# alazarteka/Self-Forcing

Measured on AMD Instinct MI355X. Metric: decoded frames/sec/node, Wan-1.3B 832x480 4-step AR rollout, higher is better.
Workload: dtype bf16

## Files before the change

### self-forcing_amd/csrc/gemm_bf16.hip

```cpp
#include <type_traits>
#include "sf_common.h"
#include "lds_dma.h"
#include "../../include/sf_hip.h"

namespace {

constexpr int BM = 128, BN = 128, BK = 64;
constexpr int GEMM_THREADS = 256;
constexpr int TILE_BYTES = BM * BK * 2;
constexpr int STAGE_BYTES = 2 * TILE_BYTES;
constexpr int GEMM_LDS = 2 * STAGE_BYTES;

struct GemmP {
  const bf16_t* a;
  const bf16_t* w;
  const bf16_t* bias;
  bf16_t* out;
  const bf16_t* resid;
  const bf16_t* gate_mod;
  const bf16_t* gate_e0;
  long gate_group_stride;
  int rows_per_group;
  int M, N, K, lda, ldw, ldo, ldr;
  int tiles_m, tiles_n;
  long a_bs, w_bs, o_bs, r_bs;
  const float* a_scale;
  const float* w_scale;
  int rows_per_seg;
};

typedef int i32x4 __attribute__((ext_vector_type(4)));
typedef int i32x8 __attribute__((ext_vector_type(8)));

__device__ __forceinline__ f32x4 mfma_f8(const bf16x8& w0, const bf16x8& w1, const bf16x8& x0, const bf16x8& x1, const f32x4& acc) {
  const i32x8 wv = __builtin_shufflevector(__builtin_bit_cast(i32x4, w0), __builtin_bit_cast(i32x4, w1), 0, 1, 2, 3, 4, 5, 6, 7);
  const i32x8 xv = __builtin_shufflevector(__builtin_bit_cast(i32x4, x0), __builtin_bit_cast(i32x4, x1), 0, 1, 2, 3, 4, 5, 6, 7);
  return __builtin_amdgcn_mfma_scale_f32_16x16x128_f8f6f4(wv, xv, acc, 0, 0, 0, 127, 0, 127);
}

template <int MT>
__device__ __forceinline__ void fp8_scale_acc(const GemmP& p, f32x4 (&acc)[MT][4], int m_base, int n_base, int lane) {
  f32x4 ws[4];
#pragma unroll
  for (int nt = 0; nt < 4; ++nt) ws[nt] = *reinterpret_cast<const f32x4*>(p.w_scale + min(n_base + nt * 16 + (lane >> 4) * 4, p.N - 4));
#pragma unroll
  for (int mt = 0; mt < MT; ++mt) {
    const float sa = p.a_scale[min(m_base + mt * 16 + (lane & 15), p.M - 1) / p.rows_per_seg];
#pragma unroll
    for (int nt = 0; nt < 4; ++nt)
#pragma unroll
      for (int j = 0; j < 4; ++j) acc[mt][nt][j] = acc[mt][nt][j] * (sa * ws[nt][j]);
  }
}

template <int EPI>
__device__ __forceinline__ bf16x4 epi_apply(const GemmP& p, const f32x4& a4, int m, int n, const bf16_t* e0row) {
  float y[4];
#pragma unroll
  for (int j = 0; j < 4; ++j) y[j] = a4[j];
  if (p.bias) {
    const bf16x4 b = *reinterpret_cast<const bf16x4*>(p.bias + n);
#pragma unroll
    for (int j = 0; j < 4; ++j) y[j] += (float)b[j];
  }
  if (EPI == SF_EPI_BIAS_GELU) {
#pragma unroll
    for (int j = 0; j < 4; ++j) y[j] = gelu_tanh_f(y[j]);
  }
  if (EPI == SF_EPI_BIAS_GATE_RESID) {
    const bf16x4 gm = *reinterpret_cast<const bf16x4*>(p.gate_mod + n);
    const bf16x4 ge = *reinterpret_cast<const bf16x4*>(e0row + n);
#pragma unroll
    for (int j = 0; j < 4; ++j) y[j] *= (float)(bf16_t)((float)gm[j] + (float)ge[j]);
  }
  if (EPI == SF_EPI_BIAS_RESID || EPI == SF_EPI_BIAS_GATE_RESID) {
    const bf16x4 rv = *reinterpret_cast<const bf16x4*>(p.resid + (long)m * p.ldr + n);
#pragma unroll
    for (int j = 0; j < 4; ++j) y[j] += (float)rv[j];
  }
  bf16x4 o;
#pragma unroll
  for (int j = 0; j < 4; ++j) o[j] = (bf16_t)y[j];
  return o;
}

template <int EPI, int MT>
__device__ __forceinline__ void gemm_epilogue(const GemmP& p, f32x4 (&acc)[MT][4], int mrow, int ncol) {
#pragma unroll
  for (int mt = 0; mt < MT; ++mt) {
    const int m = mrow + mt * 16;
    if (m >= p.M) continue;
    const bf16_t* e0row = nullptr;
    if (EPI == SF_EPI_BIAS_GATE_RESID) e0row = p.gate_e0 + (long)(m / p.rows_per_group) * p.gate_group_stride;
#pragma unroll
    for (int nt = 0; nt < 4; ++nt) {
      const int n = ncol + nt * 16;
      if (n >= p.N) continue;
      if (EPI == SF_EPI_F32) {
        *reinterpret_cast<f32x4*>(reinterpret_cast<float*>(p.out) + (long)m * p.ldo + n) = acc[mt][nt];
        continue;
      }
      *reinterpret_cast<bf16x4*>(p.out + (long)m * p.ldo + n) = epi_apply<EPI>(p, acc[mt][nt], m, n, e0row);
    }
  }
}

template <int EPI>
__device__ __forceinline__ bf16x4 epi_math(const f32x4& a4, const bf16x4& b, const bf16x4& gm, const bf16x4& ge, const bf16x4& rv) {
  float y[4];
#pragma unroll
  for (int j = 0; j < 4; ++j) y[j] = a4[j] + (float)b[j];
  if (EPI == SF_EPI_BIAS_GELU) {
#pragma unroll
    for (int j = 0; j < 4; ++j) y[j] = gelu_tanh_f(y[j]);
  }
  if (EPI == SF_EPI_BIAS_GATE_RESID) {
#pragma unroll
    for (int j = 0; j < 4; ++j) y[j] *= (float)(bf16_t)((float)gm[j] + (float)ge[j]);
  }
  if (EPI == SF_EPI_BIAS_RESID || EPI == SF_EPI_BIAS_GATE_RESID) {
#pragma unroll
    for (int j = 0; j < 4; ++j) y[j] += (float)rv[j];
  }
  bf16x4 o;
#pragma unroll
  for (int j = 0; j < 4; ++j) o[j] = (bf16_t)y[j];
  return o;
}

template <int EPI, int MT>
__device__ __forceinline__ void gemm_epilogue_lds(const GemmP& p, f32x4 (&acc)[MT][4], int m_base, int n_base, char* wbuf, int lane) {
  const int r16 = lane & 15, cg = lane >> 4;
  constexpr bool GATE = EPI == SF_EPI_BIAS_GATE_RESID;
  constexpr bool RESID = EPI == SF_EPI_BIAS_RESID || EPI == SF_EPI_BIAS_GATE_RESID;
  const bf16x4 zero4 = {(bf16_t)0.f, (bf16_t)0.f, (bf16_t)0.f, (bf16_t)0.f};
  int ncol[4];
  bf16x4 bias_v[4], gm_v[4];
#pragma unroll
  for (int nt = 0; nt < 4; ++nt) {
    ncol[nt] = min(n_base + nt * 16 + cg * 4, p.N - 4);
    bias_v[nt] = zero4;
    gm_v[nt] = zero4;
  }
  if (p.bias) {
#pragma unroll
    for (int nt = 0; nt < 4; ++nt) bias_v[nt] = *reinterpret_cast<const bf16x4*>(p.bias + ncol[nt]);
  }
  if (GATE) {
#pragma unroll
    for (int nt = 0; nt < 4; ++nt) gm_v[nt] = *reinterpret_cast<const bf16x4*>(p.gate_mod + ncol[nt]);
  }
  constexpr int MB = 4;
#pragma unroll
  for (int m0 = 0; m0 < MT; m0 += MB) {
    bf16x4 rv[MB][4], ge[MB][4];
#pragma unroll
    for (int i = 0; i < MB; ++i) {
      if (m0 + i >= MT) break;
      const int m = min(m_base + (m0 + i) * 16 + r16, p.M - 1);
      const bf16_t* e0row = GATE ? p.gate_e0 + (long)(m / p.rows_per_group) * p.gate_group_stride : nullptr;
#pragma unroll
      for (int nt = 0; nt < 4; ++nt) {
        rv[i][nt] = RESID ? *reinterpret_cast<const bf16x4*>(p.resid + (long)m * p.ldr + ncol[nt]) : zero4;
        ge[i][nt] = GATE ? *reinterpret_cast<const bf16x4*>(e0row + ncol[nt]) : zero4;
      }
    }
#pragma unroll
    for (int i = 0; i < MB; ++i) {
      if (m0 + i >= MT) break;
      const int row = (m0 + i) * 16 + r16;
#pragma unroll
      for (int nt = 0; nt < 4; ++nt) {
        const int col = nt * 16 + cg * 4;
        const bf16x4 o = epi_math<EPI>(acc[m0 + i][nt], bias_v[nt], gm_v[nt], ge[i][nt], rv[i][nt]);
        const int chunk = (col >> 3) ^ (row & 7);
        *reinterpret_cast<bf16x4*>(wbuf + row * 128 + (chunk << 4) + (col & 4) * 2) = o;
      }
    }
  }
  __builtin_amdgcn_s_waitcnt(0xc07f);
  const int rr = lane >> 3, ch = lane & 7;
#pragma unroll
  for (int i = 0; i < 2 * MT; ++i) {
    const int row = i * 8 + rr;
    const int m = m_base + row, n = n_base + ch * 8;
    const bf16x8 v = *reinterpret_cast<const bf16x8*>(wbuf + row * 128 + ((ch ^ (row & 7)) << 4));
    if (m < p.M && n < p.N) *reinterpret_cast<bf16x8*>(p.out + (long)m * p.ldo + n) = v;
  }
}

template <int EPI, bool F8>
__global__ __launch_bounds__(GEMM_THREADS, 2) void gemm_bf16_kernel(GemmP p) {
  extern __shared__ __attribute__((aligned(16))) char smem[];
  const int tid = threadIdx.x;
  const int lane = tid & 63;
  const int wave = __builtin_amdgcn_readfirstlane(tid >> 6);

  if (blockIdx.y) {
    const long bz = blockIdx.y;
    p.a += bz * p.a_bs; p.w += bz * p.w_bs;
    if (EPI == SF_EPI_F32) p.out = reinterpret_cast<bf16_t*>(reinterpret_cast<float*>(p.out) + bz * p.o_bs); else p.out += bz * p.o_bs;
    if (p.resid) p.resid += bz * p.r_bs;
  }
  const int nwg = gridDim.x, bid = blockIdx.x;
  const int wg = sf_xcd_remap(bid, nwg);
  constexpr int GROUP_M = 8;
  const int width = GROUP_M * p.tiles_n;
  const int group = wg / width, first_m = group * GROUP_M;
  const int gsz = min(p.tiles_m - first_m, GROUP_M);
  const int in_group = wg - group * width;
  const int tm = first_m + in_group % gsz, tn = in_group / gsz;
  const int m0 = tm * BM, n0 = tn * BN;

  const bf16_t* a_src[4];
  const bf16_t* w_src[4];
#pragma unroll
  for (int i = 0; i < 4; ++i) {
    const int r = (wave * 4 + i) * 8 + (lane >> 3);
    const int c = (lane & 7) ^ ((r >> 1) & 7);
    const int am = min(m0 + r, p.M - 1);
    const int wn = min(n0 + r, p.N - 1);
    a_src[i] = p.a + (long)am * p.lda + c * 8;
    w_src[i] = p.w + (long)wn * p.ldw + c * 8;
  }
  auto stage = [&](int buf, int kt) {
    char* base = smem + buf * STAGE_BYTES + wave * 4096;
    const int k0 = kt * BK;
#pragma unroll
    for (int i = 0; i < 4; ++i) glds16(a_src[i] + k0, base + i * 1024);
#pragma unroll
    for (int i = 0; i < 4; ++i) glds16(w_src[i] + k0, base + TILE_BYTES + i * 1024);
  };

  const int wr = wave >> 1, wc = wave & 1;
  const int i16 = lane & 15, kq = lane >> 4;
  const int swz = (i16 >> 1) & 7;
  const int x_row_off = (wr * 64 + i16) * 128;
  const int w_row_off = TILE_BYTES + (wc * 64 + i16) * 128;
  const int coff0 = ((0 + kq) ^ swz) << 4;
  const int coff1 = ((4 + kq) ^ swz) << 4;

  f32x4 acc[4][4];
#pragma unroll
  for (int i = 0; i < 4; ++i)
#pragma unroll
    for (int j = 0; j < 4; ++j) acc[i][j] = f32x4{0.f, 0.f, 0.f, 0.f};

  const int nk = p.K / BK;
  stage(0, 0);
  __builtin_amdgcn_s_waitcnt(0);
  __syncthreads();

  for (int kt = 0; kt < nk; ++kt) {
    const int cur = kt & 1;
    const char* buf = smem + cur * STAGE_BYTES;
    const int kn = min(kt + 1, nk - 1) * BK;
    char* sbase = smem + (cur ^ 1) * STAGE_BYTES + wave * 4096;
    bf16x8 xf0[4], wf0[4], xf1[4], wf1[4];
    if constexpr (F8) {
#pragma unroll
      for (int t = 0; t < 4; ++t) {
        xf0[t] = *reinterpret_cast<const bf16x8*>(buf + x_row_off + t * 2048 + coff0);
        wf0[t] = *reinterpret_cast<const bf16x8*>(buf + w_row_off + t * 2048 + coff0);
        xf1[t] = *reinterpret_cast<const bf16x8*>(buf + x_row_off + t * 2048 + coff1);
        wf1[t] = *reinterpret_cast<const bf16x8*>(buf + w_row_off + t * 2048 + coff1);
      }
      __builtin_amdgcn_sched_barrier(0);
#pragma unroll
      for (int i = 0; i < 8; ++i) {
        const int mt = i >> 1, nt0 = (i & 1) * 2;
        acc[mt][nt0] = mfma_f8(wf0[nt0], wf1[nt0], xf0[mt], xf1[mt], acc[mt][nt0]);
        acc[mt][nt0 + 1] = mfma_f8(wf0[nt0 + 1], wf1[nt0 + 1], xf0[mt], xf1[mt], acc[mt][nt0 + 1]);
        if (i < 4) glds16(a_src[i] + kn, sbase + i * 1024);
        else glds16(w_src[i - 4] + kn, sbase + TILE_BYTES + (i - 4) * 1024);
        __builtin_amdgcn_sched_barrier(0);
      }
      __syncthreads();
      continue;
    }
#pragma unroll
    for (int t = 0; t < 4; ++t) {
      xf0[t] = *reinterpret_cast<const bf16x8*>(buf + x_row_off + t * 2048 + coff0);
      wf0[t] = *reinterpret_cast<const bf16x8*>(buf + w_row_off + t * 2048 + coff0);
    }
    __builtin_amdgcn_sched_barrier(0);
#pragma unroll
    for (int i = 0; i < 8; ++i) {
      const int mt = i >> 1, nt0 = (i & 1) * 2;
      acc[mt][nt0] = __builtin_amdgcn_mfma_f32_16x16x32_bf16(wf0[nt0], xf0[mt], acc[mt][nt0], 0, 0, 0);
      acc[mt][nt0 + 1] = __builtin_amdgcn_mfma_f32_16x16x32_bf16(wf0[nt0 + 1], xf0[mt], acc[mt][nt0 + 1], 0, 0, 0);
      if (i < 4) {
        xf1[i] = *reinterpret_cast<const bf16x8*>(buf + x_row_off + i * 2048 + coff1);
        glds16(a_src[i] + kn, sbase + i * 1024);
      } else {
        wf1[i - 4] = *reinterpret_cast<const bf16x8*>(buf + w_row_off + (i - 4) * 2048 + coff1);
        glds16(w_src[i - 4] + kn, sbase + TILE_BYTES + (i - 4) * 1024);
      }
      __builtin_amdgcn_sched_barrier(0);
    }
#pragma unroll
    for (int mt = 0; mt < 4; ++mt)
#pragma unroll
      for (int nt = 0; nt < 4; ++nt)
        acc[mt][nt] = __builtin_amdgcn_mfma_f32_16x16x32_bf16(wf1[nt], xf1[mt], acc[mt][nt], 0, 0, 0);
    __builtin_amdgcn_sched_barrier(0);
    __syncthreads();
  }

  if constexpr (F8) fp8_scale_acc<4>(p, acc, m0 + wr * 64, n0 + wc * 64, lane);
  const int mrow = m0 + wr * 64 + (lane & 15);
  const int ncol = n0 + wc * 64 + (lane >> 4) * 4;
  if (EPI != SF_EPI_F32 && (p.N & 7) == 0 && (p.ldo & 7) == 0)
    gemm_epilogue_lds<EPI, 4>(p, acc, m0 + wr * 64, n0 + wc * 64, smem + wave * 8192, lane);
  else
    gemm_epilogue<EPI, 4>(p, acc, mrow, ncol);
}


constexpr int PP_THREADS = 512;

template <int MT>
struct PPCfg {
  static constexpr int BM = 32 * MT;
  static constexpr int A_BYTES = BM * 128;
  static constexpr int B_BYTES = 256 * 128;
  static constexpr int STAGE = A_BYTES + B_BYTES;
  static constexpr int LDS = 2 * STAGE;
  static constexpr int PA = (2 * MT + 7) / 8;
};

template <int EPI, int MT, bool F8>
__global__ __launch_bounds__(PP_THREADS) void gemm_pp_kernel(GemmP p) {
  using Cfg = PPCfg<MT>;
  constexpr int BMp = Cfg::BM, PA = Cfg::PA;
  constexpr int HQA = (MT + 1) / 2, HQB = MT / 2;
  extern __shared__ __attribute__((aligned(16))) char smem[];
  const int tid = threadIdx.x;
  const int lane = tid & 63;
  const int wave = __builtin_amdgcn_readfirstlane(tid >> 6);
  const int grp = wave >> 2, wc = wave & 3;

  const int nwg = gridDim.x, bid = blockIdx.x;
  const int wg = sf_xcd_remap(bid, nwg);
  constexpr int GROUP_M = MT >= 6 ? 4 : 8;
  const int width = GROUP_M * p.tiles_n;
  const int group = wg / width, first_m = group * GROUP_M;
  const int gsz = min(p.tiles_m - first_m, GROUP_M);
  const int in_group = wg - group * width;
  const int tm = first_m + in_group % gsz, tn = in_group / gsz;
  const int m0 = tm * BMp, n0 = tn * 256;

  const bf16_t* a_src[2][PA];
  const bf16_t* w_src[2][2];
#pragma unroll
  for (int h = 0; h < 2; ++h) {
#pragma unroll
    for (int i = 0; i < PA; ++i) {
      const int r = h * (BMp / 2) + (wave + 8 * i) * 8 + (lane >> 3);
      const int c = (lane & 7) ^ ((r >> 1) & 7);
      a_src[h][i] = p.a + (long)min(m0 + r, p.M - 1) * p.lda + c * 8;
    }
#pragma unroll
    for (int i = 0; i < 2; ++i) {
      const int r = h * 128 + (wave + 8 * i) * 8 + (lane >> 3);
      const int c = (lane & 7) ^ ((r >> 1) & 7);
      w_src[h][i] = p.w + (long)min(n0 + r, p.N - 1) * p.ldw + c * 8;
    }
  }
  auto dma_a = [&](int h, int kt) {
    char* base = smem + (kt & 1) * Cfg::STAGE + h * (Cfg::A_BYTES / 2) + wave * 1024;
#pragma unroll
    for (int i = 0; i < PA; ++i)
      if (wave + 8 * i < 2 * MT) glds16(a_src[h][i] + kt * BK, base + i * 8192);
  };
  auto dma_b = [&](int h, int kt) {
    char* base = smem + (kt & 1) * Cfg::STAGE + Cfg::A_BYTES + h * (Cfg::B_BYTES / 2) + wave * 1024;
#pragma unroll
    for (int i = 0; i < 2; ++i) glds16(w_src[h][i] + kt * BK, base + i * 8192);
  };

  const int i16 = lane & 15, kq = lane >> 4;
  const int swz = (i16 >> 1) & 7;
  const int x_row_off = (grp * (BMp / 2) + i16) * 128;
  const int w_row_off = Cfg::A_BYTES + (wc * 64 + i16) * 128;
  const int coff[2] = {((0 + kq) ^ swz) << 4, ((4 + kq) ^ swz) << 4};

  f32x4 acc[MT][4];
#pragma unroll
  for (int i = 0; i < MT; ++i)
#pragma unroll
    for (int j = 0; j < 4; ++j) acc[i][j] = f32x4{0.f, 0.f, 0.f, 0.f};
  bf16x8 af[HQA][2], bfr[4][2];

#ifdef SF_STAMP
  unsigned long long* stamp = (EPI == SF_EPI_BIAS && p.gate_e0) ? reinterpret_cast<unsigned long long*>(const_cast<bf16_t*>(p.gate_e0)) + ((long)bid * 2 + grp) * 8 : nullptr;
  if (stamp && (tid & 255) == 0) { stamp[0] = __builtin_amdgcn_s_memtime(); stamp[4] = __builtin_amdgcn_s_memrealtime(); }
#endif
  const int nk = p.K / BK;
  dma_a(0, 0); dma_a(1, 0); dma_b(0, 0); dma_b(1, 0);
  if (nk > 1) { dma_b(0, 1); dma_b(1, 1); asm volatile("s_waitcnt vmcnt(4)" ::: "memory"); }
  else asm volatile("s_waitcnt vmcnt(0)" ::: "memory");
  __builtin_amdgcn_s_barrier();
#ifdef SF_STAMP
  if (stamp && (tid & 255) == 0) stamp[1] = __builtin_amdgcn_s_memtime();
#endif
  if (grp == 1) __builtin_amdgcn_s_barrier();

  auto end_load_segment = [&]() {
    __builtin_amdgcn_s_waitcnt(0xc07f);
    __builtin_amdgcn_sched_barrier(0);
    __builtin_amdgcn_s_barrier();
    __builtin_amdgcn_sched_barrier(0);
  };
  auto cluster = [&](auto qc, int c0) {
    constexpr int q = decltype(qc)::value, NQ = q == 0 ? HQA : HQB;
    __builtin_amdgcn_s_setprio(1);
    if constexpr (F8) {
#pragma unroll
      for (int mt = 0; mt < NQ; ++mt)
#pragma unroll
        for (int nt = 0; nt < 2; ++nt)
          acc[q * HQA + mt][c0 + nt] = mfma_f8(bfr[c0 + nt][0], bfr[c0 + nt][1], af[mt][0], af[mt][1], acc[q * HQA + mt][c0 + nt]);
    } else {
#pragma unroll
      for (int ks = 0; ks < 2; ++ks)
#pragma unroll
        for (int mt = 0; mt < NQ; ++mt)
#pragma unroll
          for (int nt = 0; nt < 2; ++nt)
            acc[q * HQA + mt][c0 + nt] = __builtin_amdgcn_mfma_f32_16x16x32_bf16(bfr[c0 + nt][ks], af[mt][ks], acc[q * HQA + mt][c0 + nt], 0, 0, 0);
    }
    __builtin_amdgcn_s_setprio(0);
    __builtin_amdgcn_sched_barrier(0);
    __builtin_amdgcn_s_barrier();
    __builtin_amdgcn_sched_barrier(0);
  };
  auto read_a = [&](const char* buf, auto qc) {
    constexpr int q = decltype(qc)::value, NQ = q == 0 ? HQA : HQB;
#pragma unroll
    for (int mt = 0; mt < NQ; ++mt)
#pragma unroll
      for (int ks = 0; ks < 2; ++ks)
        af[mt][ks] = *reinterpret_cast<const bf16x8*>(buf + x_row_off + (q * HQA + mt) * 2048 + coff[ks]);
  };
  auto read_b = [&](const char* buf, int c0) {
#pragma unroll
    for (int nt = 0; nt < 2; ++nt)
#pragma unroll
      for (int ks = 0; ks < 2; ++ks)
        bfr[c0 + nt][ks] = *reinterpret_cast<const bf16x8*>(buf + w_row_off + (c0 + nt) * 2048 + coff[ks]);
  };

  constexpr std::integral_constant<int, 0> Q0{};
  constexpr std::integral_constant<int, 1> Q1{};
  for (int kt = 0; kt < nk; ++kt) {
    const char* buf = smem + (kt & 1) * Cfg::STAGE;
    const bool more1 = kt + 1 < nk, more2 = kt + 2 < nk;
    read_a(buf, Q0);
    read_b(buf, 0);
    if (more1) dma_a(0, kt + 1);
    end_load_segment();
    cluster(Q0, 0);
    read_b(buf, 2);
    if (more1) dma_a(1, kt + 1);
    end_load_segment();
    cluster(Q0, 2);
    read_a(buf, Q1);
    if (more2) dma_b(0, kt + 2);
    end_load_segment();
    cluster(Q1, 2);
    if (more2) {
      dma_b(1, kt + 2);
      asm volatile("s_waitcnt vmcnt(4)" ::: "memory");
    } else {
      asm volatile("s_waitcnt vmcnt(0)" ::: "memory");
    }
    end_load_segment();
    cluster(Q1, 0);
  }
  if (grp == 0) __builtin_amdgcn_s_barrier();
#ifdef SF_STAMP
  if (stamp && (tid & 255) == 0) stamp[2] = __builtin_amdgcn_s_memtime();
#endif

  const int m_base = m0 + grp * (BMp / 2), n_base = n0 + wc * 64;
  if constexpr (F8) fp8_scale_acc<MT>(p, acc, m_base, n_base, lane);
  if ((p.N & 7) == 0 && (p.ldo & 7) == 0)
    gemm_epilogue_lds<EPI, MT>(p, acc, m_base, n_base, smem + wave * (MT * 2048), lane);
  else
    gemm_epilogue<EPI, MT>(p, acc, m_base + (lane & 15), n_base + (lane >> 4) * 4);
#ifdef SF_STAMP
  asm volatile("s_waitcnt vmcnt(0)" ::: "memory");
  if (stamp && (tid & 255) == 0) { stamp[3] = __builtin_amdgcn_s_memtime(); stamp[5] = __builtin_amdgcn_s_memrealtime(); }
#endif
}

constexpr int PP2_A = 128 * 128, PP2_B = 256 * 128;
constexpr int PP2_LDS = 3 * (PP2_A + PP2_B);

template <int EPI, bool F8>
__global__ __launch_bounds__(PP_THREADS) void gemm_pp2_kernel(GemmP p) {
  extern __shared__ __attribute__((aligned(16))) char smem[];
  const int tid = threadIdx.x;
  const int lane = tid & 63;
  const int wave = __builtin_amdgcn_readfirstlane(tid >> 6);
  const int grp = wave >> 2, wc = wave & 3;

  const int nwg = gridDim.x, bid = blockIdx.x;
  const int wg = sf_xcd_remap(bid, nwg);
  constexpr int GROUP_M = 8;
  const int width = GROUP_M * p.tiles_n;
  const int group = wg / width, first_m = group * GROUP_M;
  const int gsz = min(p.tiles_m - first_m, GROUP_M);
  const int in_group = wg - group * width;
  const int tm = first_m + in_group % gsz, tn = in_group / gsz;
  const int m0 = tm * 128, n0 = tn * 256;

  const bf16_t* a_src[2];
  const bf16_t* w_src[4];
#pragma unroll
  for (int i = 0; i < 2; ++i) {
    const int r = (wave + 8 * i) * 8 + (lane >> 3);
    a_src[i] = p.a + (long)min(m0 + r, p.M - 1) * p.lda + ((lane & 7) ^ ((r >> 1) & 7)) * 8;
  }
#pragma unroll
  for (int i = 0; i < 4; ++i) {
    const int r = (wave + 8 * i) * 8 + (lane >> 3);
    w_src[i] = p.w + (long)min(n0 + r, p.N - 1) * p.ldw + ((lane & 7) ^ ((r >> 1) & 7)) * 8;
  }
  auto dma_a = [&](int slot, int kt) {
    char* base = smem + slot * PP2_A + wave * 1024;
#pragma unroll
    for (int i = 0; i < 2; ++i) glds16(a_src[i] + kt * BK, base + i * 8192);
  };
  auto dma_b = [&](int slot, int kt) {
    char* base = smem + 3 * PP2_A + slot * PP2_B + wave * 1024;
#pragma unroll
    for (int i = 0; i < 4; ++i) glds16(w_src[i] + kt * BK, base + i * 8192);
  };

  const int i16 = lane & 15, kq = lane >> 4;
  const int swz = (i16 >> 1) & 7;
  const int x_row_off = (grp * 64 + i16) * 128;
  const int w_row_off = 3 * PP2_A + (wc * 64 + i16) * 128;
  const int coff[2] = {((0 + kq) ^ swz) << 4, ((4 + kq) ^ swz) << 4};

  f32x4 acc[4][4];
#pragma unroll
  for (int i = 0; i < 4; ++i)
#pragma unroll
    for (int j = 0; j < 4; ++j) acc[i][j] = f32x4{0.f, 0.f, 0.f, 0.f};
  bf16x8 af[4][2], bfr[4][2];

  const int nk = p.K / BK;
  dma_a(0, 0); dma_b(0, 0);
  if (nk > 1) { dma_a(1, 1); dma_b(1, 1); asm volatile("s_waitcnt vmcnt(6)" ::: "memory"); }
  else asm volatile("s_waitcnt vmcnt(0)" ::: "memory");
  __builtin_amdgcn_s_barrier();
  if (grp == 1) __builtin_amdgcn_s_barrier();

  auto end_load_segment = [&]() {
    __builtin_amdgcn_s_waitcnt(0xc07f);
    __builtin_amdgcn_sched_barrier(0);
    __builtin_amdgcn_s_barrier();
    __builtin_amdgcn_sched_barrier(0);
  };
  auto cluster = [&](int c0) {
    __builtin_amdgcn_s_setprio(1);
    if constexpr (F8) {
#pragma unroll
      for (int mt = 0; mt < 4; ++mt)
#pragma unroll
        for (int nt = 0; nt < 2; ++nt)
          acc[mt][c0 + nt] = mfma_f8(bfr[c0 + nt][0], bfr[c0 + nt][1], af[mt][0], af[mt][1], acc[mt][c0 + nt]);
    } else {
#pragma unroll
      for (int ks = 0; ks < 2; ++ks)
#pragma unroll
        for (int mt = 0; mt < 4; ++mt)
#pragma unroll
          for (int nt = 0; nt < 2; ++nt)
            acc[mt][c0 + nt] = __builtin_amdgcn_mfma_f32_16x16x32_bf16(bfr[c0 + nt][ks], af[mt][ks], acc[mt][c0 + nt], 0, 0, 0);
    }
    __builtin_amdgcn_s_setprio(0);
    __builtin_amdgcn_sched_barrier(0);
    __builtin_amdgcn_s_barrier();
    __builtin_amdgcn_sched_barrier(0);
  };

  int slot = 0;
  for (int kt = 0; kt < nk; ++kt) {
    const char* abuf = smem + slot * PP2_A;
    const char* bbuf = smem + slot * PP2_B;
    const int nslot = slot == 0 ? 2 : slot - 1;
    const bool more2 = kt + 2 < nk;
#pragma unroll
    for (int mt = 0; mt < 4; ++mt)
#pragma unroll
      for (int ks = 0; ks < 2; ++ks) af[mt][ks] = *reinterpret_cast<const bf16x8*>(abuf + x_row_off + mt * 2048 + coff[ks]);
#pragma unroll
    for (int nt = 0; nt < 2; ++nt)
#pragma unroll
      for (int ks = 0; ks < 2; ++ks) bfr[nt][ks] = *reinterpret_cast<const bf16x8*>(bbuf + w_row_off + nt * 2048 + coff[ks]);
    if (more2) dma_a(nslot, kt + 2);
    end_load_segment();
    cluster(0);
#pragma unroll
    for (int nt = 2; nt < 4; ++nt)
#pragma unroll
      for (int ks = 0; ks < 2; ++ks) bfr[nt][ks] = *reinterpret_cast<const bf16x8*>(bbuf + w_row_off + nt * 2048 + coff[ks]);
    if (more2) {
      dma_b(nslot, kt + 2);
      asm volatile("s_waitcnt vmcnt(6)" ::: "memory");
    } else {
      asm volatile("s_waitcnt vmcnt(0)" ::: "memory");
    }
    end_load_segment();
    cluster(2);
    slot = slot == 2 ? 0 : slot + 1;
  }
  if (grp == 0) __builtin_amdgcn_s_barrier();

  const int m_base = m0 + grp * 64, n_base = n0 + wc * 64;
  if constexpr (F8) fp8_scale_acc<4>(p, acc, m_base, n_base, lane);
  if ((p.N & 7) == 0 && (p.ldo & 7) == 0)
    gemm_epilogue_lds<EPI, 4>(p, acc, m_base, n_base, smem + wave * 8192, lane);
  else
    gemm_epilogue<EPI, 4>(p, acc, m_base + (lane & 15), n_base + (lane >> 4) * 4);
}

template <int EPI, bool F8>
int launch_pp2(GemmP& p, hipStream_t s) {
  static bool attr = false;
  if (!attr) {
    (void)hipFuncSetAttribute(reinterpret_cast<const void*>(&gemm_pp2_kernel<EPI, F8>), hipFuncAttributeMaxDynamicSharedMemorySize, PP2_LDS);
    attr = true;
  }
  p.tiles_m = (p.M + 127) / 128;
  p.tiles_n = (p.N + 255) / 256;
  hipLaunchKernelGGL((gemm_pp2_kernel<EPI, F8>), dim3(p.tiles_m * p.tiles_n), dim3(PP_THREADS), PP2_LDS, s, p);
  return 0;
}

template <bool F8>
int launch_pp2_epi(GemmP& p, int epilogue, hipStream_t s) {
  switch (epilogue) {
    case SF_EPI_BIAS: return launch_pp2<SF_EPI_BIAS, F8>(p, s);
    case SF_EPI_BIAS_GELU: return launch_pp2<SF_EPI_BIAS_GELU, F8>(p, s);
    case SF_EPI_BIAS_RESID: return launch_pp2<SF_EPI_BIAS_RESID, F8>(p, s);
    case SF_EPI_BIAS_GATE_RESID: return launch_pp2<SF_EPI_BIAS_GATE_RESID, F8>(p, s);
    default: return -1;
  }
}

template <int EPI, int MT, bool F8>
int launch_pp(GemmP& p, hipStream_t s) {
  using Cfg = PPCfg<MT>;
  static bool attr = false;
  if (!attr) {
    (void)hipFuncSetAttribute(reinterpret_cast<const void*>(&gemm_pp_kernel<EPI, MT, F8>), hipFuncAttributeMaxDynamicSharedMemorySize, Cfg::LDS);
    attr = true;
  }
  p.tiles_m = (p.M + Cfg::BM - 1) / Cfg::BM;
  p.tiles_n = (p.N + 255) / 256;
  hipLaunchKernelGGL((gemm_pp_kernel<EPI, MT, F8>), dim3(p.tiles_m * p.tiles_n), dim3(PP_THREADS), Cfg::LDS, s, p);
  return 0;
}

template <int MT, bool F8>
int launch_pp_epi(GemmP& p, int epilogue, hipStream_t s) {
  switch (epilogue) {
    case SF_EPI_BIAS: return launch_pp<SF_EPI_BIAS, MT, F8>(p, s);
    case SF_EPI_BIAS_GELU: return launch_pp<SF_EPI_BIAS_GELU, MT, F8>(p, s);
    case SF_EPI_BIAS_RESID: return launch_pp<SF_EPI_BIAS_RESID, MT, F8>(p, s);
    case SF_EPI_BIAS_GATE_RESID: return launch_pp<SF_EPI_BIAS_GATE_RESID, MT, F8>(p, s);
    default: return -1;
  }
}

int check_args(const sf_gemm_args* a, const char* name, int bk) {
  SF_CHECK(a != nullptr, "%s: null args", name);
  SF_CHECK(a->M > 0 && a->N > 0 && a->K > 0, "%s: empty problem M=%d N=%d K=%d", name, a->M, a->N, a->K);
  SF_CHECK(a->K % bk == 0, "%s: K=%d must be a multiple of %d", name, a->K, bk);
  SF_CHECK(a->N % 4 == 0, "%s: N=%d must be a multiple of 4", name, a->N);
  SF_CHECK(a->lda % (bk / 8) == 0 && a->ldw % (bk / 8) == 0 && a->ldo % 4 == 0, "%s: lda/ldw must be multiples of %d, ldo of 4", name, bk / 8);
  SF_CHECK(a->lda >= a->K && a->ldw >= a->K && a->ldo >= a->N, "%s: leading dimension too small", name);
  SF_CHECK(a->a && a->w && a->out, "%s: null tensor", name);
  SF_CHECK(((uintptr_t)a->a % 16 == 0) && ((uintptr_t)a->w % 16 == 0) && ((uintptr_t)a->out % 8 == 0), "%s: misaligned tensor", name);
  if (a->epilogue == SF_EPI_BIAS_RESID || a->epilogue == SF_EPI_BIAS_GATE_RESID) {
    SF_CHECK(a->resid != nullptr && a->ldr >= a->N && a->ldr % 4 == 0, "%s: residual epilogue needs resid/ldr", name);
  }
  if (a->epilogue == SF_EPI_BIAS_GATE_RESID) {
    SF_CHECK(a->gate_mod && a->gate_e0 && a->rows_per_group > 0, "%s: gate epilogue needs gate_mod/gate_e0/rows_per_group", name);
  }
  SF_CHECK(a->structure >= SF_GEMM_AUTO && a->structure <= SF_GEMM_PP192, "%s: unknown structure %d", name, a->structure);
  return 0;
}

template <bool F8>
int run_gemm(const sf_gemm_args* a, GemmP& p, const char* name, hipStream_t s) {
  int st = a->structure;
  const int nk = p.K / BK;
  const bool pp_ok = a->batch <= 1 && a->epilogue != SF_EPI_F32 && nk >= 2;
  if (st == SF_GEMM_AUTO) {
    st = SF_GEMM_T128;
    if (pp_ok && a->M >= 1024 && a->N >= 1024 && a->K >= 512) {
      static const struct { int st, rows; double rel; } cand[] = {
          {SF_GEMM_PP256, 256, 1.00}, {SF_GEMM_PP224, 224, 1.02}, {SF_GEMM_PP192, 192, 1.05}, {SF_GEMM_PP128, 128, 1.14}};
      const long tn = (a->N + 255) / 256;
      double best = 1e30;
      for (const auto& c : cand) {
        const long tiles = (long)((a->M + c.rows - 1) / c.rows) * tn;
        const double cost = (double)((tiles + 255) / 256) * (c.rows / 256.0 * c.rel + 0.04);
        if (cost < best - 1e-9) { best = cost; st = c.st; }
      }
    }
  }
  const bool is_pp = st == SF_GEMM_PP256 || st == SF_GEMM_PP224 || st == SF_GEMM_PP192 || st == SF_GEMM_PP128;
  if (is_pp && !pp_ok) st = SF_GEMM_T128;
  else if (is_pp) {
    const int rc = st == SF_GEMM_PP256 ? launch_pp_epi<8, F8>(p, a->epilogue, s)
                 : st == SF_GEMM_PP224 ? launch_pp_epi<7, F8>(p, a->epilogue, s)
                 : st == SF_GEMM_PP192 ? launch_pp_epi<6, F8>(p, a->epilogue, s) : launch_pp2_epi<F8>(p, a->epilogue, s);
    SF_CHECK(rc == 0, "%s: unknown epilogue %d", name, a->epilogue);
    SF_HIP_LAUNCH_CHECK(name);
    return 0;
  }
  const int batch = a->batch > 1 ? a->batch : 1;
  p.a_bs = a->a_bstride; p.w_bs = a->w_bstride; p.o_bs = a->o_bstride; p.r_bs = a->r_bstride;
  SF_CHECK(batch == 1 || (a->a_bstride % 8 == 0 && a->w_bstride % 8 == 0 && a->o_bstride % 4 == 0 && a->r_bstride % 4 == 0),
           "%s: batch strides must keep 16-byte (operands) / 8-byte (output) alignment", name);
  const dim3 grid(p.tiles_m * p.tiles_n, batch), block(GEMM_THREADS);
  switch (a->epilogue) {
    case SF_EPI_BIAS: hipLaunchKernelGGL((gemm_bf16_kernel<SF_EPI_BIAS, F8>), grid, block, GEMM_LDS, s, p); break;
    case SF_EPI_BIAS_GELU: hipLaunchKernelGGL((gemm_bf16_kernel<SF_EPI_BIAS_GELU, F8>), grid, block, GEMM_LDS, s, p); break;
    case SF_EPI_BIAS_RESID: hipLaunchKernelGGL((gemm_bf16_kernel<SF_EPI_BIAS_RESID, F8>), grid, block, GEMM_LDS, s, p); break;
    case SF_EPI_BIAS_GATE_RESID: hipLaunchKernelGGL((gemm_bf16_kernel<SF_EPI_BIAS_GATE_RESID, F8>), grid, block, GEMM_LDS, s, p); break;
    case SF_EPI_F32:
      if constexpr (F8) {
        SF_CHECK(false, "%s: the raw fp32 epilogue is bf16-only", name);
      } else {
        SF_CHECK((uintptr_t)a->out % 16 == 0, "%s: fp32 output must be 16-byte aligned", name);
        hipLaunchKernelGGL((gemm_bf16_kernel<SF_EPI_F32, false>), grid, block, GEMM_LDS, s, p);
      }
      break;
    default: SF_CHECK(false, "%s: unknown epilogue %d", name, a->epilogue);
  }
  SF_HIP_LAUNCH_CHECK(name);
  return 0;
}

void fill_params(const sf_gemm_args* a, GemmP& p, int unit) {
  p.a = (const bf16_t*)a->a; p.w = (const bf16_t*)a->w; p.bias = (const bf16_t*)a->bias;
  p.out = (bf16_t*)a->out; p.resid = (const bf16_t*)a->resid;
  p.gate_mod = (const bf16_t*)a->gate_mod; p.gate_e0 = (const bf16_t*)a->gate_e0;
  p.gate_group_stride = a->gate_group_stride; p.rows_per_group = a->rows_per_group;
  p.M = a->M; p.N = a->N; p.K = a->K / unit; p.lda = a->lda / unit; p.ldw = a->ldw / unit; p.ldo = a->ldo; p.ldr = a->ldr;
  p.tiles_n = (a->N + BN - 1) / BN;
  p.tiles_m = (a->M + BM - 1) / BM;
  p.a_scale = nullptr; p.w_scale = nullptr; p.rows_per_seg = 1;
}

}

extern "C" int sf_gemm_bf16(const sf_gemm_args* a, void* stream) {
  if (const int rc = check_args(a, "sf_gemm_bf16", BK)) return rc;
  GemmP p;
  fill_params(a, p, 1);
  return run_gemm<false>(a, p, "sf_gemm_bf16", (hipStream_t)stream);
}

extern "C" int sf_gemm_fp8(const sf_gemm_args* a, const float* a_scale, int rows_per_segment, const float* w_scale, void* stream) {
  if (const int rc = check_args(a, "sf_gemm_fp8", 2 * BK)) return rc;
  SF_CHECK(a->batch <= 1, "sf_gemm_fp8: batched products are bf16-only");
  SF_CHECK(a_scale && w_scale && rows_per_segment > 0, "sf_gemm_fp8: needs a_scale, w_scale and rows_per_segment > 0");
  SF_CHECK((uintptr_t)w_scale % 16 == 0, "sf_gemm_fp8: w_scale must be 16-byte aligned");
  GemmP p;
  fill_params(a, p, 2);
  p.a_scale = a_scale; p.w_scale = w_scale; p.rows_per_seg = rows_per_segment;
  return run_gemm<true>(a, p, "sf_gemm_fp8", (hipStream_t)stream);
}
```

Before: 93.76.

## Prefetch GEMM epilogue operands during final K-tile and hoist gate computation

Bias, gate and residual loads for the LDS epilogue are now issued early: column operands before the K loop, and residual rows in place of DMA slots during the peeled last K iteration. This hides epilogue global-load latency behind the final MFMAs. The gate (mod + e0) is formed once per row group instead of once per row, with a loop over groups when a tile spans several. The cost is higher register pressure and more template and scheduling complexity (opaque asm, sched barriers).

```diff
diff --git a/self-forcing_amd/csrc/gemm_bf16.hip b/self-forcing_amd/csrc/gemm_bf16.hip
--- a/self-forcing_amd/csrc/gemm_bf16.hip
+++ b/self-forcing_amd/csrc/gemm_bf16.hip
@@ -32,6 +32,14 @@
 typedef int i32x4 __attribute__((ext_vector_type(4)));
 typedef int i32x8 __attribute__((ext_vector_type(8)));
 
+template <int N, int I = 0, class F>
+__device__ __forceinline__ void static_for(F&& f) {
+  if constexpr (I < N) {
+    f(std::integral_constant<int, I>{});
+    static_for<N, I + 1>(f);
+  }
+}
+
 __device__ __forceinline__ f32x4 mfma_f8(const bf16x8& w0, const bf16x8& w1, const bf16x8& x0, const bf16x8& x1, const f32x4& acc) {
   const i32x8 wv = __builtin_shufflevector(__builtin_bit_cast(i32x4, w0), __builtin_bit_cast(i32x4, w1), 0, 1, 2, 3, 4, 5, 6, 7);
   const i32x8 xv = __builtin_shufflevector(__builtin_bit_cast(i32x4, x0), __builtin_bit_cast(i32x4, x1), 0, 1, 2, 3, 4, 5, 6, 7);
@@ -106,7 +114,7 @@
 }
 
 template <int EPI>
-__device__ __forceinline__ bf16x4 epi_math(const f32x4& a4, const bf16x4& b, const bf16x4& gm, const bf16x4& ge, const bf16x4& rv) {
+__device__ __forceinline__ bf16x4 epi_math(const f32x4& a4, const bf16x4& b, const bf16x4& g, const bf16x4& rv) {
   float y[4];
 #pragma unroll
   for (int j = 0; j < 4; ++j) y[j] = a4[j] + (float)b[j];
@@ -116,7 +124,7 @@
   }
   if (EPI == SF_EPI_BIAS_GATE_RESID) {
 #pragma unroll
-    for (int j = 0; j < 4; ++j) y[j] *= (float)(bf16_t)((float)gm[j] + (float)ge[j]);
+    for (int j = 0; j < 4; ++j) y[j] *= (float)g[j];
   }
   if (EPI == SF_EPI_BIAS_RESID || EPI == SF_EPI_BIAS_GATE_RESID) {
 #pragma unroll
@@ -128,55 +136,139 @@
   return o;
 }
 
+__device__ __forceinline__ void opaque(f32x4& v) { asm volatile("" : "+v"(v)); }
+__device__ __forceinline__ void opaque(bf16x4& v) {
+  unsigned long long t = __builtin_bit_cast(unsigned long long, v);
+  asm volatile("" : "+v"(t));
+  v = __builtin_bit_cast(bf16x4, t);
+}
+
+__device__ __forceinline__ bf16x4 epi_gate(const bf16x4& gm, const bf16x4& ge) {
+  bf16x4 g;
+#pragma unroll
+  for (int j = 0; j < 4; ++j) g[j] = (bf16_t)((float)gm[j] + (float)ge[j]);
+  return g;
+}
+
 template <int EPI, int MT>
-__device__ __forceinline__ void gemm_epilogue_lds(const GemmP& p, f32x4 (&acc)[MT][4], int m_base, int n_base, char* wbuf, int lane) {
+struct EpiOps {
+  static constexpr bool GATE = EPI == SF_EPI_BIAS_GATE_RESID;
+  static constexpr bool RESID = EPI == SF_EPI_BIAS_RESID || EPI == SF_EPI_BIAS_GATE_RESID;
+  int ncol[4];
+  bf16x4 bias[4];
+  bf16x4 gate[4];
+  bf16x4 ge[4];
+  bf16x4 rv[MT][4];
+  int g_first, g_last;
+};
+
+template <int EPI, int MT>
+__device__ __forceinline__ void epi_request_cols(const GemmP& p, EpiOps<EPI, MT>& e, int m_base, int n_base, int lane) {
+  const bf16x4 zero4 = {(bf16_t)0.f, (bf16_t)0.f, (bf16_t)0.f, (bf16_t)0.f};
+  const int cg = lane >> 4;
+#pragma unroll
+  for (int nt = 0; nt < 4; ++nt) {
+    e.ncol[nt] = min(n_base + nt * 16 + cg * 4, p.N - 4);
+    e.bias[nt] = zero4;
+    e.gate[nt] = zero4;
+  }
+  e.g_first = e.g_last = 0;
+  if constexpr (!EpiOps<EPI, MT>::RESID) {
+#pragma unroll
+    for (int b = 0; b < MT; ++b)
+#pragma unroll
+      for (int nt = 0; nt < 4; ++nt) e.rv[b][nt] = zero4;
+  }
+  if (p.bias) {
+#pragma unroll
+    for (int nt = 0; nt < 4; ++nt) e.bias[nt] = *reinterpret_cast<const bf16x4*>(p.bias + e.ncol[nt]);
+  }
+  if constexpr (EpiOps<EPI, MT>::GATE) {
+#pragma unroll
+    for (int nt = 0; nt < 4; ++nt) e.gate[nt] = *reinterpret_cast<const bf16x4*>(p.gate_mod + e.ncol[nt]);
+    e.g_first = min(m_base, p.M - 1) / p.rows_per_group;
+    e.g_last = min(m_base + 16 * MT - 1, p.M - 1) / p.rows_per_group;
+    const bf16_t* e0row = p.gate_e0 + (long)e.g_first * p.gate_group_stride;
+#pragma unroll
+    for (int nt = 0; nt < 4; ++nt) e.ge[nt] = *reinterpret_cast<const bf16x4*>(e0row + e.ncol[nt]);
+  }
+}
+
+template <int EPI, int MT>
+__device__ __forceinline__ void epi_form_gate(EpiOps<EPI, MT>& e) {
+  if constexpr (EpiOps<EPI, MT>::GATE) {
+#pragma unroll
+    for (int nt = 0; nt < 4; ++nt) e.gate[nt] = epi_gate(e.gate[nt], e.ge[nt]);
+  }
+#pragma unroll
+  for (int nt = 0; nt < 4; ++nt) opaque(e.bias[nt]);
+}
+
+template <int B0, int B1, int EPI, int MT>
+__device__ __forceinline__ void epi_request_rows(const GemmP& p, EpiOps<EPI, MT>& e, int m_base, int lane) {
+  if constexpr (EpiOps<EPI, MT>::RESID) {
+#pragma unroll
+    for (int b = B0; b < (B1 < MT ? B1 : MT); ++b) {
+      const bf16_t* rrow = p.resid + (long)min(m_base + b * 16 + (lane & 15), p.M - 1) * p.ldr;
+#pragma unroll
+      for (int nt = 0; nt < 4; ++nt) e.rv[b][nt] = *reinterpret_cast<const bf16x4*>(rrow + e.ncol[nt]);
+    }
+  }
+}
+
+template <int MT, bool F8> struct EpiPlan {
+  static constexpr bool EARLY = !(F8 && MT == 8);
+  static constexpr int PRE = !EARLY ? 4 : (MT == 8 || (F8 && MT == 7)) ? 2 : MT < 4 ? MT : 4, HALF = (PRE + 1) / 2;
+  static constexpr int WIN = EARLY ? MT : 4;
+};
+
+template <int EPI, int MT, int PRE, int WIN = MT>
+__device__ __forceinline__ void gemm_epilogue_lds(const GemmP& p, f32x4 (&acc)[MT][4], EpiOps<EPI, MT>& e, int m_base, int n_base, char* wbuf, int lane) {
   const int r16 = lane & 15, cg = lane >> 4;
-  constexpr bool GATE = EPI == SF_EPI_BIAS_GATE_RESID;
-  constexpr bool RESID = EPI == SF_EPI_BIAS_RESID || EPI == SF_EPI_BIAS_GATE_RESID;
-  const bf16x4 zero4 = {(bf16_t)0.f, (bf16_t)0.f, (bf16_t)0.f, (bf16_t)0.f};
-  int ncol[4];
-  bf16x4 bias_v[4], gm_v[4];
-#pragma unroll
-  for (int nt = 0; nt < 4; ++nt) {
-    ncol[nt] = min(n_base + nt * 16 + cg * 4, p.N - 4);
-    bias_v[nt] = zero4;
-    gm_v[nt] = zero4;
-  }
-  if (p.bias) {
-#pragma unroll
-    for (int nt = 0; nt < 4; ++nt) bias_v[nt] = *reinterpret_cast<const bf16x4*>(p.bias + ncol[nt]);
-  }
-  if (GATE) {
-#pragma unroll
-    for (int nt = 0; nt < 4; ++nt) gm_v[nt] = *reinterpret_cast<const bf16x4*>(p.gate_mod + ncol[nt]);
-  }
-  constexpr int MB = 4;
-#pragma unroll
-  for (int m0 = 0; m0 < MT; m0 += MB) {
-    bf16x4 rv[MB][4], ge[MB][4];
-#pragma unroll
-    for (int i = 0; i < MB; ++i) {
-      if (m0 + i >= MT) break;
-      const int m = min(m_base + (m0 + i) * 16 + r16, p.M - 1);
-      const bf16_t* e0row = GATE ? p.gate_e0 + (long)(m / p.rows_per_group) * p.gate_group_stride : nullptr;
-#pragma unroll
-      for (int nt = 0; nt < 4; ++nt) {
-        rv[i][nt] = RESID ? *reinterpret_cast<const bf16x4*>(p.resid + (long)m * p.ldr + ncol[nt]) : zero4;
-        ge[i][nt] = GATE ? *reinterpret_cast<const bf16x4*>(e0row + ncol[nt]) : zero4;
-      }
-    }
-#pragma unroll
-    for (int i = 0; i < MB; ++i) {
-      if (m0 + i >= MT) break;
-      const int row = (m0 + i) * 16 + r16;
+  constexpr bool GATE = EpiOps<EPI, MT>::GATE;
+  __builtin_amdgcn_sched_barrier(0);
+  if constexpr (EpiOps<EPI, MT>::RESID && PRE > 0 && PRE < WIN) {
+#pragma unroll
+    for (int b = 0; b < PRE; ++b)
+#pragma unroll
+      for (int nt = 0; nt < 4; ++nt) opaque(e.rv[b][nt]);
+    __builtin_amdgcn_sched_barrier(0);
+  }
+  epi_request_rows<PRE, WIN>(p, e, m_base, lane);
+  __builtin_amdgcn_sched_barrier(0);
+  for (int g = e.g_first;;) {
+    static_for<MT>([&](auto ic) {
+      constexpr int i = decltype(ic)::value;
+      const int row = i * 16 + r16;
+      bool mine = true;
+      if constexpr (GATE) {
+        if (e.g_first != e.g_last) {
+          const int lo = g * p.rows_per_group - m_base, hi = lo + p.rows_per_group;
+          if (i * 16 >= hi || i * 16 + 15 < lo) return;
+          mine = r16 >= lo - i * 16 && r16 < hi - i * 16;
+        }
+      }
 #pragma unroll
       for (int nt = 0; nt < 4; ++nt) {
         const int col = nt * 16 + cg * 4;
-        const bf16x4 o = epi_math<EPI>(acc[m0 + i][nt], bias_v[nt], gm_v[nt], ge[i][nt], rv[i][nt]);
+        if constexpr (GATE) { opaque(acc[i][nt]); opaque(e.rv[i][nt]); opaque(e.bias[nt]); }
+        const bf16x4 o = epi_math<EPI>(acc[i][nt], e.bias[nt], e.gate[nt], e.rv[i][nt]);
         const int chunk = (col >> 3) ^ (row & 7);
-        *reinterpret_cast<bf16x4*>(wbuf + row * 128 + (chunk << 4) + (col & 4) * 2) = o;
-      }
-    }
+        if (mine) *reinterpret_cast<bf16x4*>(wbuf + row * 128 + (chunk << 4) + (col & 4) * 2) = o;
+      }
+      __builtin_amdgcn_sched_barrier(0);
+      if constexpr (WIN < MT) {
+        __builtin_amdgcn_sched_barrier(0);
+        epi_request_rows<i + WIN, i + WIN + 1>(p, e, m_base, lane);
+        __builtin_amdgcn_sched_barrier(0);
+      }
+    });
+    if (!GATE || g == e.g_last) break;
+    ++g;
+    const bf16_t* e0row = p.gate_e0 + (long)g * p.gate_group_stride;
+#pragma unroll
+    for (int nt = 0; nt < 4; ++nt)
+      e.gate[nt] = epi_gate(*reinterpret_cast<const bf16x4*>(p.gate_mod + e.ncol[nt]), *reinterpret_cast<const bf16x4*>(e0row + e.ncol[nt]));
   }
   __builtin_amdgcn_s_waitcnt(0xc07f);
   const int rr = lane >> 3, ch = lane & 7;
@@ -246,16 +338,42 @@
 #pragma unroll
     for (int j = 0; j < 4; ++j) acc[i][j] = f32x4{0.f, 0.f, 0.f, 0.f};
 
+  const int em_base = m0 + wr * 64, en_base = n0 + wc * 64;
+  const bool lds_epi = EPI != SF_EPI_F32 && (p.N & 7) == 0 && (p.ldo & 7) == 0;
+  EpiOps<EPI, 4> eo;
+  if (lds_epi) epi_request_cols(p, eo, em_base, en_base, lane);
+
   const int nk = p.K / BK;
   stage(0, 0);
   __builtin_amdgcn_s_waitcnt(0);
   __syncthreads();
-
-  for (int kt = 0; kt < nk; ++kt) {
+  if (lds_epi) epi_form_gate(eo);
+
+  auto kstep = [&](int kt, auto lastc) {
+    constexpr bool LAST = decltype(lastc)::value;
     const int cur = kt & 1;
     const char* buf = smem + cur * STAGE_BYTES;
-    const int kn = min(kt + 1, nk - 1) * BK;
+    const int kn = (kt + 1) * BK;
     char* sbase = smem + (cur ^ 1) * STAGE_BYTES + wave * 4096;
+    auto request = [&](auto ic) {
+      constexpr int i = decltype(ic)::value;
+      if constexpr (!LAST) {
+        if constexpr (i < 4) glds16(a_src[i] + kn, sbase + i * 1024);
+        else glds16(w_src[i - 4] + kn, sbase + TILE_BYTES + (i - 4) * 1024);
+      } else if constexpr (i < 4) {
+        if (lds_epi) epi_request_rows<i, i + 1>(p, eo, em_base, lane);
+      }
+    };
+    auto end_step = [&]() {
+      if constexpr (LAST) {
+        __builtin_amdgcn_s_waitcnt(0xc07f);
+        __builtin_amdgcn_sched_barrier(0);
+        __builtin_amdgcn_s_barrier();
+        __builtin_amdgcn_sched_barrier(0);
+      } else {
+        __syncthreads();
+      }
+    };
     bf16x8 xf0[4], wf0[4], xf1[4], wf1[4];
     if constexpr (F8) {
 #pragma unroll
@@ -266,17 +384,16 @@
         wf1[t] = *reinterpret_cast<const bf16x8*>(buf + w_row_off + t * 2048 + coff1);
       }
       __builtin_amdgcn_sched_barrier(0);
-#pragma unroll
-      for (int i = 0; i < 8; ++i) {
-        const int mt = i >> 1, nt0 = (i & 1) * 2;
+      static_for<8>([&](auto ic) {
+        constexpr int i = decltype(ic)::value;
+        constexpr int mt = i >> 1, nt0 = (i & 1) * 2;
         acc[mt][nt0] = mfma_f8(wf0[nt0], wf1[nt0], xf0[mt], xf1[mt], acc[mt][nt0]);
         acc[mt][nt0 + 1] = mfma_f8(wf0[nt0 + 1], wf1[nt0 + 1], xf0[mt], xf1[mt], acc[mt][nt0 + 1]);
-        if (i < 4) glds16(a_src[i] + kn, sbase + i * 1024);
-        else glds16(w_src[i - 4] + kn, sbase + TILE_BYTES + (i - 4) * 1024);
+        request(ic);
         __builtin_amdgcn_sched_barrier(0);
-      }
-      __syncthreads();
-      continue;
+      });
+      end_step();
+      return;
     }
 #pragma unroll
     for (int t = 0; t < 4; ++t) {
@@ -284,36 +401,35 @@
       wf0[t] = *reinterpret_cast<const bf16x8*>(buf + w_row_off + t * 2048 + coff0);
     }
     __builtin_amdgcn_sched_barrier(0);
-#pragma unroll
-    for (int i = 0; i < 8; ++i) {
-      const int mt = i >> 1, nt0 = (i & 1) * 2;
+    static_for<8>([&](auto ic) {
+      constexpr int i = decltype(ic)::value;
+      constexpr int mt = i >> 1, nt0 = (i & 1) * 2;
       acc[mt][nt0] = __builtin_amdgcn_mfma_f32_16x16x32_bf16(wf0[nt0], xf0[mt], acc[mt][nt0], 0, 0, 0);
       acc[mt][nt0 + 1] = __builtin_amdgcn_mfma_f32_16x16x32_bf16(wf0[nt0 + 1], xf0[mt], acc[mt][nt0 + 1], 0, 0, 0);
-      if (i < 4) {
-        xf1[i] = *reinterpret_cast<const bf16x8*>(buf + x_row_off + i * 2048 + coff1);
-        glds16(a_src[i] + kn, sbase + i * 1024);
-      } else {
-        wf1[i - 4] = *reinterpret_cast<const bf16x8*>(buf + w_row_off + (i - 4) * 2048 + coff1);
-        glds16(w_src[i - 4] + kn, sbase + TILE_BYTES + (i - 4) * 1024);
-      }
+      if constexpr (i < 4) xf1[i] = *reinterpret_cast<const bf16x8*>(buf + x_row_off + i * 2048 + coff1);
+      else wf1[i - 4] = *reinterpret_cast<const bf16x8*>(buf + w_row_off + (i - 4) * 2048 + coff1);
+      request(ic);
       __builtin_amdgcn_sched_barrier(0);
-    }
+    });
 #pragma unroll
     for (int mt = 0; mt < 4; ++mt)
 #pragma unroll
       for (int nt = 0; nt < 4; ++nt)
         acc[mt][nt] = __builtin_amdgcn_mfma_f32_16x16x32_bf16(wf1[nt], xf1[mt], acc[mt][nt], 0, 0, 0);
     __builtin_amdgcn_sched_barrier(0);
-    __syncthreads();
-  }
-
-  if constexpr (F8) fp8_scale_acc<4>(p, acc, m0 + wr * 64, n0 + wc * 64, lane);
-  const int mrow = m0 + wr * 64 + (lane & 15);
-  const int ncol = n0 + wc * 64 + (lane >> 4) * 4;
-  if (EPI != SF_EPI_F32 && (p.N & 7) == 0 && (p.ldo & 7) == 0)
-    gemm_epilogue_lds<EPI, 4>(p, acc, m0 + wr * 64, n0 + wc * 64, smem + wave * 8192, lane);
-  else
-    gemm_epilogue<EPI, 4>(p, acc, mrow, ncol);
+    end_step();
+  };
+  for (int kt = 0; kt < nk - 1; ++kt) kstep(kt, std::false_type{});
+  kstep(nk - 1, std::true_type{});
+
+  if constexpr (F8) fp8_scale_acc<4>(p, acc, em_base, en_base, lane);
+  if constexpr (EPI != SF_EPI_F32) {
+    if (lds_epi) {
+      gemm_epilogue_lds<EPI, 4, 4>(p, acc, eo, em_base, en_base, smem + wave * 8192, lane);
+      return;
+    }
+  }
+  gemm_epilogue<EPI, 4>(p, acc, em_base + (lane & 15), en_base + (lane >> 4) * 4);
 }
 
 
@@ -396,6 +512,12 @@
   unsigned long long* stamp = (EPI == SF_EPI_BIAS && p.gate_e0) ? reinterpret_cast<unsigned long long*>(const_cast<bf16_t*>(p.gate_e0)) + ((long)bid * 2 + grp) * 8 : nullptr;
   if (stamp && (tid & 255) == 0) { stamp[0] = __builtin_amdgcn_s_memtime(); stamp[4] = __builtin_amdgcn_s_memrealtime(); }
 #endif
+  const int m_base = m0 + grp * (BMp / 2), n_base = n0 + wc * 64;
+  const bool lds_epi = (p.N & 7) == 0 && (p.ldo & 7) == 0;
+  using Plan = EpiPlan<MT, F8>;
+  EpiOps<EPI, MT> eo;
+  if (Plan::EARLY && lds_epi) epi_request_cols(p, eo, m_base, n_base, lane);
+
   const int nk = p.K / BK;
   dma_a(0, 0); dma_a(1, 0); dma_b(0, 0); dma_b(1, 0);
   if (nk > 1) { dma_b(0, 1); dma_b(1, 1); asm volatile("s_waitcnt vmcnt(4)" ::: "memory"); }
@@ -404,6 +526,7 @@
 #ifdef SF_STAMP
   if (stamp && (tid & 255) == 0) stamp[1] = __builtin_amdgcn_s_memtime();
 #endif
+  if (Plan::EARLY && lds_epi) epi_form_gate(eo);
   if (grp == 1) __builtin_amdgcn_s_barrier();
 
   auto end_load_segment = [&]() {
@@ -421,6 +544,10 @@
 #pragma unroll
         for (int nt = 0; nt < 2; ++nt)
           acc[q * HQA + mt][c0 + nt] = mfma_f8(bfr[c0 + nt][0], bfr[c0 + nt][1], af[mt][0], af[mt][1], acc[q * HQA + mt][c0 + nt]);
+#pragma unroll
+      for (int mt = 0; mt < NQ; ++mt)
+#pragma unroll
+        for (int nt = 0; nt < 2; ++nt) opaque(acc[q * HQA + mt][c0 + nt]);
     } else {
 #pragma unroll
       for (int ks = 0; ks < 2; ++ks)
@@ -453,40 +580,53 @@
 
   constexpr std::integral_constant<int, 0> Q0{};
   constexpr std::integral_constant<int, 1> Q1{};
-  for (int kt = 0; kt < nk; ++kt) {
+  constexpr int RPRE = Plan::PRE, RHALF = Plan::HALF;
+  auto tile = [&](int kt, auto lastc) {
+    constexpr bool LAST = decltype(lastc)::value;
     const char* buf = smem + (kt & 1) * Cfg::STAGE;
-    const bool more1 = kt + 1 < nk, more2 = kt + 2 < nk;
+    const bool more2 = kt + 2 < nk;
     read_a(buf, Q0);
     read_b(buf, 0);
-    if (more1) dma_a(0, kt + 1);
+    if constexpr (!LAST) dma_a(0, kt + 1);
+    else if (Plan::EARLY && lds_epi) epi_request_rows<0, RHALF>(p, eo, m_base, lane);
     end_load_segment();
     cluster(Q0, 0);
     read_b(buf, 2);
-    if (more1) dma_a(1, kt + 1);
+    if constexpr (!LAST) dma_a(1, kt + 1);
+    else if (Plan::EARLY && lds_epi) epi_request_rows<RHALF, RPRE>(p, eo, m_base, lane);
     end_load_segment();
     cluster(Q0, 2);
     read_a(buf, Q1);
-    if (more2) dma_b(0, kt + 2);
+    if constexpr (!LAST) { if (more2) dma_b(0, kt + 2); }
     end_load_segment();
     cluster(Q1, 2);
-    if (more2) {
-      dma_b(1, kt + 2);
-      asm volatile("s_waitcnt vmcnt(4)" ::: "memory");
-    } else {
-      asm volatile("s_waitcnt vmcnt(0)" ::: "memory");
+    if constexpr (!LAST) {
+      if (more2) {
+        dma_b(1, kt + 2);
+        asm volatile("s_waitcnt vmcnt(4)" ::: "memory");
+      } else {
+        asm volatile("s_waitcnt vmcnt(0)" ::: "memory");
+      }
     }
     end_load_segment();
     cluster(Q1, 0);
-  }
+  };
+  for (int kt = 0; kt < nk - 1; ++kt) tile(kt, std::false_type{});
+  tile(nk - 1, std::true_type{});
   if (grp == 0) __builtin_amdgcn_s_barrier();
 #ifdef SF_STAMP
   if (stamp && (tid & 255) == 0) stamp[2] = __builtin_amdgcn_s_memtime();
 #endif
 
-  const int m_base = m0 + grp * (BMp / 2), n_base = n0 + wc * 64;
+  if (!Plan::EARLY && lds_epi) {
+    epi_request_cols(p, eo, m_base, n_base, lane);
+    epi_request_rows<0, RPRE>(p, eo, m_base, lane);
+    __builtin_amdgcn_sched_barrier(0);
+  }
   if constexpr (F8) fp8_scale_acc<MT>(p, acc, m_base, n_base, lane);
-  if ((p.N & 7) == 0 && (p.ldo & 7) == 0)
-    gemm_epilogue_lds<EPI, MT>(p, acc, m_base, n_base, smem + wave * (MT * 2048), lane);
+  if (!Plan::EARLY && lds_epi) epi_form_gate(eo);
+  if (lds_epi)
+    gemm_epilogue_lds<EPI, MT, RPRE, Plan::WIN>(p, acc, eo, m_base, n_base, smem + wave * (MT * 2048), lane);
   else
     gemm_epilogue<EPI, MT>(p, acc, m_base + (lane & 15), n_base + (lane >> 4) * 4);
 #ifdef SF_STAMP
@@ -552,11 +692,17 @@
     for (int j = 0; j < 4; ++j) acc[i][j] = f32x4{0.f, 0.f, 0.f, 0.f};
   bf16x8 af[4][2], bfr[4][2];
 
+  const int m_base = m0 + grp * 64, n_base = n0 + wc * 64;
+  const bool lds_epi = (p.N & 7) == 0 && (p.ldo & 7) == 0;
+  EpiOps<EPI, 4> eo;
+  if (lds_epi) epi_request_cols(p, eo, m_base, n_base, lane);
+
   const int nk = p.K / BK;
   dma_a(0, 0); dma_b(0, 0);
   if (nk > 1) { dma_a(1, 1); dma_b(1, 1); asm volatile("s_waitcnt vmcnt(6)" ::: "memory"); }
   else asm volatile("s_waitcnt vmcnt(0)" ::: "memory");
   __builtin_amdgcn_s_barrier();
+  if (lds_epi) epi_form_gate(eo);
   if (grp == 1) __builtin_amdgcn_s_barrier();
 
   auto end_load_segment = [&]() {
@@ -573,6 +719,10 @@
 #pragma unroll
         for (int nt = 0; nt < 2; ++nt)
           acc[mt][c0 + nt] = mfma_f8(bfr[c0 + nt][0], bfr[c0 + nt][1], af[mt][0], af[mt][1], acc[mt][c0 + nt]);
+#pragma unroll
+      for (int mt = 0; mt < 4; ++mt)
+#pragma unroll
+        for (int nt = 0; nt < 2; ++nt) opaque(acc[mt][c0 + nt]);
     } else {
 #pragma unroll
       for (int ks = 0; ks < 2; ++ks)
@@ -589,7 +739,8 @@
   };
 
   int slot = 0;
-  for (int kt = 0; kt < nk; ++kt) {
+  auto tile = [&](int kt, auto lastc) {
+    constexpr bool LAST = decltype(lastc)::value;
     const char* abuf = smem + slot * PP2_A;
     const char* bbuf = smem + slot * PP2_B;
     const int nslot = slot == 0 ? 2 : slot - 1;
@@ -602,29 +753,35 @@
     for (int nt = 0; nt < 2; ++nt)
 #pragma unroll
       for (int ks = 0; ks < 2; ++ks) bfr[nt][ks] = *reinterpret_cast<const bf16x8*>(bbuf + w_row_off + nt * 2048 + coff[ks]);
-    if (more2) dma_a(nslot, kt + 2);
+    if constexpr (!LAST) { if (more2) dma_a(nslot, kt + 2); }
+    else if (lds_epi) epi_request_rows<0, 2>(p, eo, m_base, lane);
     end_load_segment();
     cluster(0);
 #pragma unroll
     for (int nt = 2; nt < 4; ++nt)
 #pragma unroll
       for (int ks = 0; ks < 2; ++ks) bfr[nt][ks] = *reinterpret_cast<const bf16x8*>(bbuf + w_row_off + nt * 2048 + coff[ks]);
-    if (more2) {
-      dma_b(nslot, kt + 2);
-      asm volatile("s_waitcnt vmcnt(6)" ::: "memory");
-    } else {
-      asm volatile("s_waitcnt vmcnt(0)" ::: "memory");
+    if constexpr (!LAST) {
+      if (more2) {
+        dma_b(nslot, kt + 2);
+        asm volatile("s_waitcnt vmcnt(6)" ::: "memory");
+      } else {
+        asm volatile("s_waitcnt vmcnt(0)" ::: "memory");
+      }
+    } else if (lds_epi) {
+      epi_request_rows<2, 4>(p, eo, m_base, lane);
     }
     end_load_segment();
     cluster(2);
     slot = slot == 2 ? 0 : slot + 1;
-  }
+  };
+  for (int kt = 0; kt < nk - 1; ++kt) tile(kt, std::false_type{});
+  tile(nk - 1, std::true_type{});
   if (grp == 0) __builtin_amdgcn_s_barrier();
 
-  const int m_base = m0 + grp * 64, n_base = n0 + wc * 64;
   if constexpr (F8) fp8_scale_acc<4>(p, acc, m_base, n_base, lane);
-  if ((p.N & 7) == 0 && (p.ldo & 7) == 0)
-    gemm_epilogue_lds<EPI, 4>(p, acc, m_base, n_base, smem + wave * 8192, lane);
+  if (lds_epi)
+    gemm_epilogue_lds<EPI, 4, 4>(p, acc, eo, m_base, n_base, smem + wave * 8192, lane);
   else
     gemm_epilogue<EPI, 4>(p, acc, m_base + (lane & 15), n_base + (lane >> 4) * 4);
 }
```

Measured after the change: 93.49. About the same (-0.3%).
